# locuslab/qpth

Measured on AMD Instinct MI355X. Metric: QPs/sec (fwd+bwd) at batch=512 nz=100 nineq=100; 1/2/4/8 MI355X, higher is better.
Workload: dtype f64; 1 GPU; C2 fwd+bwd: batch=512 nz=100 nineq=100 neq=0 per GPU, dense random QP (prof-linear.py generator), QPFunction(verbose=-1) defaults, p requires grad; global_batch=512, parallelism=batch-sharded x1, tensor_dtype=f64, arithmetic=f64

## Files before the change

include/qpx.h:

```cpp
#ifndef QPX_H
#define QPX_H

#include <stddef.h>
#include <stdint.h>

#ifdef __cplusplus
extern "C" {
#endif

#define QPX_ABI_VERSION 8

enum { QPX_F32 = 0, QPX_F64 = 1, QPX_F32_WIDE = 2 };

enum {
    QPX_OK = 0,
    QPX_ERR_ARG = -1,
    QPX_ERR_UNSUPPORTED = -2,
    QPX_ERR_LAUNCH = -3,
    QPX_ERR_NO_DEVICE = -4
};

enum {
    QPX_ST_Q_NOT_SPD = 1,
    QPX_ST_A_RANK = 2,
// ... 15 lines not shown
int qpx_max_dim(void);
int qpx_supported(int dtype, int n, int m, int q);
enum { QPX_FAMILY_GRID = 1, QPX_FAMILY_TILE = 2, QPX_FAMILY_BIG = 3 };
int qpx_kernel_family(int dtype, int n, int m, int q);
int qpx_refine_supported(int dtype, int n, int m, int q);

int qpx_set_ipm_variant(int variant);
int qpx_get_ipm_variant(void);

int qpx_can_share_factors(int dtype, int n, int m, int q);

int qpx_big_gemm_r(int dtype, int B, int n, int m, int q, void* factors, qpx_stream_t stream);

int qpx_pre_factor(int dtype, int B, int n, int m, int q,
                   const void* Q, int64_t sQ, const void* G, int64_t sG, const void* A, int64_t sA,
                   void* factors, int32_t* status, qpx_stream_t stream);

int qpx_ipm(int dtype, int B, int n, int m, int q,
            const void* p, int64_t sp, const void* h, int64_t sh, const void* b, int64_t sb,
            void* factors, int64_t sfac, double eps, int maxIter, int notImprovedLim, int stall_policy,
            void* zhat, void* nu, void* lam, void* slack,
            int32_t* iters, int32_t* status, void* best_resid, void* trace, qpx_stream_t stream);

int qpx_forward(int dtype, int B, int n, int m, int q,
                const void* Q, int64_t sQ, const void* p, int64_t sp,
                const void* G, int64_t sG, const void* h, int64_t sh,
                const void* A, int64_t sA, const void* b, int64_t sb,
                void* factors, double eps, int maxIter, int notImprovedLim, int stall_policy,
                void* zhat, void* nu, void* lam, void* slack,
                int32_t* iters, int32_t* status, void* best_resid, void* trace, qpx_stream_t stream);

int qpx_factor_solve_kkt(int dtype, int B, int n, int m, int q, void* factors, int64_t sfac,
                         const void* d, const void* rx, const void* rs, const void* rz, const void* ry,
                         void* dx, void* ds, void* dz, void* dy,
                         int refine, const void* Q, int64_t sQ, const void* G, int64_t sG, const void* A, int64_t sA,
                         int32_t* status, qpx_stream_t stream);

int qpx_backward(int dtype, int B, int n, int m, int q, void* factors, int64_t sfac,
                 const void* zhat, const void* lam, const void* slack, const void* nu, const void* dl_dz,
                 void* dQ, void* dp, void* dG, void* dh, void* dA, void* db,
                 void* dx, void* dz, void* dy,
                 int refine, const void* Q, int64_t sQ, const void* G, int64_t sG, const void* A, int64_t sA,
                 int32_t* status, qpx_stream_t stream);

int qpx_backward_duals(int dtype, int B, int n, int m, int q, void* factors, int64_t sfac,
                       const void* zhat, const void* lam, const void* slack, const void* nu,
// ... 39 lines not shown
```

qpth_amd/_lib.py:

```python
import ctypes
import os

import torch

_HERE = os.path.dirname(os.path.abspath(__file__))
HIP_SO = os.path.join(_HERE, "libqpx_hip.so")

QPX_F32, QPX_F64, QPX_F32_WIDE = 0, 1, 2
ST_Q_NOT_SPD, ST_A_RANK, ST_KKT_BREAKDOWN, ST_INACCURATE, ST_MAXITER, ST_NONFINITE = 1, 2, 4, 8, 16, 32
STALL_OFF, STALL_REFERENCE, STALL_FLOOR = 0, 1, 2
FAMILY_GRID, FAMILY_TILE, FAMILY_BIG = 1, 2, 3

_vp, _i, _i64, _d = ctypes.c_void_p, ctypes.c_int, ctypes.c_int64, ctypes.c_double

_SIGNATURES = {
    "qpx_abi_version": (_i, []),
    "qpx_strerror": (ctypes.c_char_p, [_i]),
    "qpx_factor_elems": (ctypes.c_size_t, [_i, _i, _i, _i]),
    "qpx_max_dim": (_i, []),
    "qpx_supported": (_i, [_i, _i, _i, _i]),
    "qpx_kernel_family": (_i, [_i, _i, _i, _i]),
    "qpx_refine_supported": (_i, [_i, _i, _i, _i]),
    "qpx_set_ipm_variant": (_i, [_i]),
    "qpx_get_ipm_variant": (_i, []),
    "qpx_can_share_factors": (_i, [_i, _i, _i, _i]),
    "qpx_big_gemm_r": (_i, [_i, _i, _i, _i, _i, _vp, _vp]),
    "qpx_pre_factor": (_i, [_i, _i, _i, _i, _i, _vp, _i64, _vp, _i64, _vp, _i64, _vp, _vp, _vp]),
    "qpx_ipm": (_i, [_i, _i, _i, _i, _i, _vp, _i64, _vp, _i64, _vp, _i64, _vp, _i64, _d, _i, _i, _i,
                     _vp, _vp, _vp, _vp, _vp, _vp, _vp, _vp, _vp]),
    "qpx_forward": (_i, [_i, _i, _i, _i, _i, _vp, _i64, _vp, _i64, _vp, _i64, _vp, _i64, _vp, _i64,
                         _vp, _i64, _vp, _d, _i, _i, _i, _vp, _vp, _vp, _vp, _vp, _vp, _vp, _vp, _vp]),
    "qpx_factor_solve_kkt": (_i, [_i, _i, _i, _i, _i, _vp, _i64, _vp, _vp, _vp, _vp, _vp, _vp, _vp, _vp, _vp,
                                  _i, _vp, _i64, _vp, _i64, _vp, _i64, _vp, _vp]),
    "qpx_backward": (_i, [_i, _i, _i, _i, _i, _vp, _i64, _vp, _vp, _vp, _vp, _vp, _vp, _vp, _vp, _vp, _vp,
                          _vp, _vp, _vp, _vp, _i, _vp, _i64, _vp, _i64, _vp, _i64, _vp, _vp]),
    "qpx_backward_duals": (_i, [_i, _i, _i, _i, _i, _vp, _i64, _vp, _vp, _vp, _vp, _vp, _vp, _vp, _vp, _vp, _vp, _vp, _vp,
                                _vp, _vp, _vp, _vp, _i, _vp, _i64, _vp, _i64, _vp, _i64, _vp, _vp]),
    "qpx_jvp": (_i, [_i, _i, _i, _i, _i, _vp, _i64, _vp, _vp, _vp, _vp, _vp, _i64, _vp, _i64, _vp, _i64, _vp, _i64,
                     _vp, _i64, _vp, _i64, _vp, _vp, _vp, _vp, _i, _vp, _i64, _vp, _i64, _vp, _i64, _vp, _vp]),
    "qpx_multi_supported": (_i, [_i, _i, _i, _i]),
    "qpx_factor_solve_kkt_multi": (_i, [_i, _i, _i, _i, _i, _i, _vp, _i64, _vp, _vp, _vp, _vp, _vp, _vp, _vp, _vp, _vp, _vp, _vp]),
    "qpx_polish_supported": (_i, [_i, _i, _i, _i]),
    "qpx_polish": (_i, [_i, _i, _i, _i, _i, _vp, _i64, _vp, _i64, _vp, _i64, _vp, _i64, _vp, _i64, _vp, _i64,
                        _vp, _i64, _i, _i, _vp, _vp, _vp, _vp, _vp, _vp, _vp]),
    "qpx_batch_outer": (_i, [_i, _i, _i, _i, _vp, _vp, _vp, _vp, _d, _vp, _vp, ctypes.c_size_t, _vp]),
    "qpx_batch_outer_workspace_elems": (ctypes.c_size_t, [_i, _i, _i, _i]),
    "qpx_dense_solve": (_i, [_i, _i, _i, _vp, _vp, _vp, _vp]),
}
ABI_SYMBOLS = tuple(_SIGNATURES)


def _dtype_code(t):
# ... 45 lines not shown
    def __init__(self, path, strict=True):
        if not os.path.exists(path):
            raise RuntimeError(
                "qpth_amd: %s is missing. Build the gfx950 extension first "
                "(python -c 'import __graft_entry__ as g; g.build()' or qpth_amd/csrc/build.sh). "
                "There is no CPU fallback." % path)
        self.path = path
        self.dll = ctypes.CDLL(path)
        for name, (res, args) in _SIGNATURES.items():
            if not strict and not hasattr(self.dll, name):
                continue
            fn = getattr(self.dll, name)
            fn.restype, fn.argtypes = res, args
        if strict and self.dll.qpx_abi_version() != 8:
            raise RuntimeError("qpth_amd: ABI version mismatch in %s" % path)

    def check(self, code):
        if code != 0:
            raise RuntimeError("qpth_amd: %s (code %d)" % (self.dll.qpx_strerror(code).decode(), code))

    def factor_elems(self, dtype_code, n, m, q):
        return int(self.dll.qpx_factor_elems(dtype_code, n, m, q))

    def pre_factor(self, B, n, m, q, Q, G, A, factors, status, wide=False):
        Qp, Gp, Ap = Param(Q, 3), Param(G, 3), Param(A, 3)
        self.check(self.dll.qpx_pre_factor(
            _code(factors, wide), B, n, m, q, Qp.ptr, Qp.stride, Gp.ptr, Gp.stride, Ap.ptr, Ap.stride,
            _ptr(factors), _ptr(status), _stream(factors)))

    def ipm(self, B, n, m, q, p, h, b, factors, sfac, eps, maxIter, notImprovedLim, stall_policy,
            zhat, nu, lam, slack, iters, status, best_resid, trace=None, wide=False):
        pp, hp, bp = Param(p, 2), Param(h, 2), Param(b, 2)
        self.check(self.dll.qpx_ipm(
            _code(factors, wide), B, n, m, q, pp.ptr, pp.stride, hp.ptr, hp.stride, bp.ptr, bp.stride,
            _ptr(factors), int(sfac), float(eps), int(maxIter), int(notImprovedLim), int(stall_policy),
            _ptr(zhat), _ptr(nu), _ptr(lam), _ptr(slack), _ptr(iters), _ptr(status), _ptr(best_resid),
            _ptr(trace), _stream(factors)))

    def forward(self, B, n, m, q, Q, p, G, h, A, b, factors, eps, maxIter, notImprovedLim,
                stall_policy, zhat, nu, lam, slack, iters, status, best_resid, trace=None, wide=False):
        Qp, Gp, Ap = Param(Q, 3), Param(G, 3), Param(A, 3)
        pp, hp, bp = Param(p, 2), Param(h, 2), Param(b, 2)
        self.check(self.dll.qpx_forward(
            _code(factors, wide), B, n, m, q, Qp.ptr, Qp.stride, pp.ptr, pp.stride, Gp.ptr, Gp.stride,
            hp.ptr, hp.stride, Ap.ptr, Ap.stride, bp.ptr, bp.stride, _ptr(factors), float(eps),
            int(maxIter), int(notImprovedLim), int(stall_policy), _ptr(zhat), _ptr(nu), _ptr(lam),
            _ptr(slack), _ptr(iters), _ptr(status), _ptr(best_resid), _ptr(trace), _stream(factors)))

    def factor_solve_kkt(self, B, n, m, q, factors, sfac, d, rx, rs, rz, ry, dx, ds, dz, dy, status,
                         refine=0, Q=None, G=None, A=None, wide=False):
        Qp, Gp, Ap = Param(Q, 3), Param(G, 3), Param(A, 3)
        self.check(self.dll.qpx_factor_solve_kkt(
            _code(factors, wide), B, n, m, q, _ptr(factors), int(sfac), _ptr(d), _ptr(rx), _ptr(rs), _ptr(rz),
            _ptr(ry), _ptr(dx), _ptr(ds), _ptr(dz), _ptr(dy), int(refine), Qp.ptr, Qp.stride, Gp.ptr, Gp.stride,
            Ap.ptr, Ap.stride, _ptr(status), _stream(factors)))
# ... 82 lines not shown
```

qpth_amd/csrc/qpx_api.inc:

```
#include "qpx_forms.h"

namespace qpx {

constexpr int kMaxDim = 1024;
constexpr int kMaxDimPolish = 512;

static thread_local int g_grid_size = 0;
static thread_local int g_ipm_variant = 0;

inline bool use_grid(int n, int m, int q)
{
    return g_ipm_variant == 0 && grid_nb(n + q + m) > 0;
}

static thread_local int g_prefac_sweep = 0;
static thread_local int g_tile_nw = 0;
inline bool tile_chain(int nbt, int nw) { return (nbt == 7 || nbt == 4) && nw == 4; }
inline int tile_waves(int nbt, int B)
{
    int nw = g_tile_nw;
    if (nw == 0) nw = nbt == 7 ? 4 : (nbt == 4 && B <= 2 * 256 ? 4 : 1);
    if (nbt == 7 && nw == 1) nw = 2;
    if (nbt <= 2) nw = 1;
    if (nbt == 4 && nw > 2) nw = 4;
// ... 22 lines not shown
    if (d <= 256) return 4;
    if (d <= 512) return 8;
    if (d <= kMaxDim) return 16;
    return 0;
}

inline int check_dims(int dtype, int B, int n, int m, int q)
{
    if (dtype != QPX_F32 && dtype != QPX_F64 && dtype != QPX_F32_WIDE) return QPX_ERR_ARG;
    if (B < 1 || n < 1 || m < 1 || q < 0) return QPX_ERR_ARG;
    if (q > n) return QPX_ERR_ARG;
    if (!slots_for(n, m, q)) return QPX_ERR_UNSUPPORTED;
    return QPX_OK;
}

template <class T> inline size_t blob_elems(int n, int m, int q)
{
    const int images = blob_images<T>(n, m, q);
    return images == 8 ? big_layout(n, m, q).total : fac_layout(n, m, q, images).total;
}

#include "qpx_big_host.inc"

template <class T>
int api_pre_factor(int B, int n, int m, int q, const void* Q, int64_t sQ, const void* G, int64_t sG,
                   const void* A, int64_t sA, void* factors, int32_t* status, void* stream, int io32 = 0)
{
    if (!Q || !G || !factors || !status || (q > 0 && !A)) return QPX_ERR_ARG;
    PrefactorArgs<T> a;
    a.io32 = io32;
    a.B = B; a.n = n; a.m = m; a.q = q;
    a.Q = (const T*)Q; a.G = (const T*)G; a.A = (const T*)A;
    a.sQ = sQ; a.sG = sG; a.sA = sA;
    a.images = blob_images<T>(n, m, q);
    if (a.images == 8) {
        const size_t fs = big_layout(n, m, q).total;
        return big_split(B, stream, true, [&](int q0, int cnt, void* st, int part, int nparts) {
            return big_pre_factor<T>(cnt, n, m, q, advio(a.Q, (size_t)q0 * sQ, io32), sQ, advio(a.G, (size_t)q0 * sG, io32), sG,
                                     advio(a.A, (size_t)q0 * sA, io32), sA, (T*)factors + (size_t)q0 * fs, status + q0, st, io32);
        });
    }
    a.fac = (T*)factors; a.fac_stride = fac_layout(n, m, q, a.images).total; a.status = status;
    if constexpr (std::is_same<T, double>::value) {
        if (use_grid(n, m, q) && !g_prefac_sweep && prefac_tile_serves(n, m, q, a.images)) {
            const int nbn = tile_nb(n + q);
            const size_t pb = lds_elems_prefac_tile(nbn, (m + 15) / 16) * sizeof(double);
            prefac_deal(nbn, n + q, m, a.pf_k, a.pf_r);
#define QPX_PICK(NBN, EQ) if (nbn == NBN && (q > 0) == EQ) return launch_prefac_tile<NBN, EQ>(a, pb, stream);
            QPX_FORMS_PREFAC_TILE(QPX_PICK)
#undef QPX_PICK
        }
    }
    if (use_grid(n, m, q)) {
        const int nba = sweep_nb(n + q + m);
        const size_t gb = lds_elems_sweep(nba) * sizeof(T);
#define QPX_PICK(NBL) if (nba == NBL) return launch_sweep<T, NBL>(a, gb, stream);
        QPX_FORMS_SWEEP(QPX_PICK)
#undef QPX_PICK
    }
    return QPX_ERR_UNSUPPORTED;
}

template <class T>
int api_ipm(int B, int n, int m, int q, const void* p, int64_t sp, const void* h, int64_t sh,
            const void* bb, int64_t sb, void* factors, int64_t sfac, double eps, int maxIter, int notImprovedLim,
            int stall_policy, void* zhat, void* nu, void* lam, void* slack, int32_t* iters,
            int32_t* status, void* best_resid, void* trace, void* stream, int io32 = 0)
{
    if (!p || !h || !factors || !zhat || !lam || !slack || !iters || !status || !best_resid ||
        (q > 0 && (!nu || !bb)))
        return QPX_ERR_ARG;
    if (maxIter < 0 || stall_policy < 0 || stall_policy > 2) return QPX_ERR_ARG;
    IpmArgs<T> a;
    a.io32 = io32;
    a.B = B; a.n = n; a.m = m; a.q = q;
    a.p = (const T*)p; a.h = (const T*)h; a.b = (const T*)bb;
    a.sp = sp; a.sh = sh; a.sb = sb;
    a.fac = (T*)factors; a.fac_stride = (size_t)sfac;
    a.eps = (T)eps; a.maxIter = maxIter; a.notImprovedLim = notImprovedLim; a.stall_policy = stall_policy;
    a.zhat = (T*)zhat; a.nu = (T*)nu; a.lam = (T*)lam; a.slack = (T*)slack;
    a.iters = iters; a.status = status; a.best_resid = (T*)best_resid; a.trace = (T*)trace;
    a.images = blob_images<T>(n, m, q);
    if (a.images == 8) {
        if (sfac == 0 && B > 1) return QPX_ERR_ARG;
        return big_split(B, stream, a.trace == nullptr, [&](int q0, int cnt, void* st, int part, int nparts) {
            IpmArgs<T> s = a;
            const size_t o = (size_t)q0;
            s.B = cnt;
            s.p = advio(a.p, o * a.sp, io32); s.h = advio(a.h, o * a.sh, io32); s.b = advio(a.b, o * a.sb, io32);
            s.fac += o * a.fac_stride;
            s.zhat = advio(a.zhat, o * n, io32); s.lam = advio(a.lam, o * m, io32); s.slack = advio(a.slack, o * m, io32);
            s.nu = advio(a.nu, o * q, io32);
            s.iters += q0; s.status += q0; s.best_resid = advio(a.best_resid, o, io32);
            return big_ipm<T>(s, st, part, nparts);
        });
    }
    if (use_grid(n, m, q)) {
// ... 287 lines not shown
    if (!factors) return QPX_ERR_ARG;
    if (!qpx::use_big(n, m, q, dtype != QPX_F32 ? 8 : 4)) return QPX_ERR_UNSUPPORTED;
    return dtype != QPX_F32 ? qpx::big_gemm_r<double>(B, n, m, (double*)factors, stream, q)
                            : qpx::big_gemm_r<float>(B, n, m, (float*)factors, stream, q);
}

int qpx_can_share_factors(int dtype, int n, int m, int q)
{
    if (qpx::check_dims(dtype, 1, n, m, q) != QPX_OK) return 0;
    return qpx::use_big(n, m, q, dtype != QPX_F32 ? 8 : 4) ? 0 : 1;
}

int qpx_pre_factor(int dtype, int B, int n, int m, int q, const void* Q, int64_t sQ, const void* G,
                   int64_t sG, const void* A, int64_t sA, void* factors, int32_t* status,
                   qpx_stream_t stream)
{
    const int e = qpx::check_dims(dtype, B, n, m, q);
    if (e) return e;
    return dtype != QPX_F32
               ? qpx::api_pre_factor<double>(B, n, m, q, Q, sQ, G, sG, A, sA, factors, status, stream, dtype == QPX_F32_WIDE)
               : qpx::api_pre_factor<float>(B, n, m, q, Q, sQ, G, sG, A, sA, factors, status, stream);
}

int qpx_ipm(int dtype, int B, int n, int m, int q, const void* p, int64_t sp, const void* h,
            int64_t sh, const void* b, int64_t sb, void* factors, int64_t sfac, double eps, int maxIter,
            int notImprovedLim, int stall_policy, void* zhat, void* nu, void* lam, void* slack,
            int32_t* iters, int32_t* status, void* best_resid, void* trace, qpx_stream_t stream)
{
    const int e = qpx::check_dims(dtype, B, n, m, q);
    if (e) return e;
    return dtype != QPX_F32
               ? qpx::api_ipm<double>(B, n, m, q, p, sp, h, sh, b, sb, factors, sfac, eps, maxIter, notImprovedLim, stall_policy, zhat, nu, lam, slack, iters, status, best_resid, trace, stream, dtype == QPX_F32_WIDE)
               : qpx::api_ipm<float>(B, n, m, q, p, sp, h, sh, b, sb, factors, sfac, eps, maxIter, notImprovedLim, stall_policy, zhat, nu, lam, slack, iters, status, best_resid, trace, stream);
}

int qpx_forward(int dtype, int B, int n, int m, int q, const void* Q, int64_t sQ, const void* p,
                int64_t sp, const void* G, int64_t sG, const void* h, int64_t sh, const void* A,
                int64_t sA, const void* b, int64_t sb, void* factors, double eps, int maxIter,
                int notImprovedLim, int stall_policy, void* zhat, void* nu, void* lam, void* slack,
                int32_t* iters, int32_t* status, void* best_resid, void* trace, qpx_stream_t stream)
{
    int e = qpx_pre_factor(dtype, B, n, m, q, Q, sQ, G, sG, A, sA, factors, status, stream);
    if (e) return e;
    return qpx_ipm(dtype, B, n, m, q, p, sp, h, sh, b, sb, factors, (int64_t)qpx_factor_elems(dtype, n, m, q), eps, maxIter, notImprovedLim,
                   stall_policy, zhat, nu, lam, slack, iters, status, best_resid, trace, stream);
}
// ... 141 lines not shown
```

qpth_amd/csrc/qpx_grid.h:

```cpp
#pragma once
#include "qpx_forms.h"
#include "qpx_kernels.h"

namespace qpx {

template <int I0, int N, class F> QPX_DEV void static_for_(F&& f)
{
    if constexpr (I0 < N) {
        f(std::integral_constant<int, I0>{});
        static_for_<I0 + 1, N>(f);
    }
}
template <int N, class F> QPX_DEV void static_for(F&& f) { static_for_<0, N>(f); }

constexpr int gtri(int x) { return x * (x + 1) / 2; }
constexpr int gidx(int li, int lj) { return li * (li + 1) / 2 + lj; }

template <int GS> struct GridPos {
    int tid, a, b;
    static constexpr int NT = GS * GS;
    QPX_DEV explicit GridPos(const Block& blk) : tid(blk.tid), a(blk.tid % GS), b(blk.tid / GS) {}
    QPX_DEV void assign(const Block&, int*) {}
    QPX_DEV bool lead(const Block& blk) const { return blk.wave() == 0; }
    static QPX_DEV void sync(const Block& blk)
// ... 782 lines not shown

    const int lane = b.lane();
    const bool w0 = g.lead(b);
    const T mT = (T)m;
    const int io32 = a.io32;
    const In<T> pg(a.p, (size_t)qp * a.sp, io32), hg(a.h, (size_t)qp * a.sh, io32);
    const In<T> bg(q > 0 ? a.b : nullptr, (size_t)qp * a.sb, io32);

    if (a.status[qp] & (QPX_ST_Q_NOT_SPD | QPX_ST_A_RANK)) {
        const T nanv = Lim<T>::inf() - Lim<T>::inf();
        for (int i = b.tid; i < n; i += b.nt) put_(a.zhat, io32, (size_t)qp * n + i, nanv);
        for (int i = b.tid; i < m; i += b.nt) {
            put_(a.lam, io32, (size_t)qp * m + i, nanv);
            put_(a.slack, io32, (size_t)qp * m + i, nanv);
        }
        for (int i = b.tid; i < q; i += b.nt) put_(a.nu, io32, (size_t)qp * q + i, nanv);
        if (b.tid == 0) {
            a.iters[qp] = 0;
            put_(a.best_resid, io32, (size_t)qp, Lim<T>::inf());
        }
        return;
    }
    QPX_PROF_INIT
    for (int i = b.tid; i < n; i += NT) vP[i] = pg[i];
    for (int i = b.tid; i < M8; i += NT) {
        vC[i] = (i < m) ? hg[i] : T(0);
        vD[i] = T(1);
        vA[i] = T(1);
    }
    Mat::sync(b);
    block_matTvec2<T, 1, 0>(b, vC, F + lay.MT, m, vX0, F + lay.Kneg, n, vP, n);
    if (q > 0) {
        Mat::sync(b);
        for (int i = b.tid; i < q; i += NT) vTm[i] = bg[i];
        Mat::sync(b);
        for (int j = b.tid; j < m; j += NT) {
            T acc = vC[j];
            for (int r = 0; r < q; ++r) acc = fma_(-F[lay.W + (size_t)j * q + r], vTm[r], acc);
            vC[j] = acc;
        }
    }
    Mat::sync(b);
    QPX_PROF(0)

    typename Mat::Regs E;
    enum { kTau = 0, kBtau, kSigz, kSigs, kBres, kFeasPrev, kAlphaPrev, kMu, kSzdot, kFeas, kResid, kGt1 };
    enum { kStop = 0, kNnot, kFloor, kSt, kIters };
    if (b.tid == 0) {
        sc[kTau] = T(1); sc[kBtau] = T(1); sc[kSigz] = T(0); sc[kSigs] = T(0); sc[kBres] = Lim<T>::inf();
        sc[kFeasPrev] = T(0); sc[kAlphaPrev] = T(0);
        sc[kGt1] = F[lay.scal];
        ctrl[kStop] = 0; ctrl[kNnot] = 0; ctrl[kFloor] = 0; ctrl[kSt] = 0; ctrl[kIters] = 0;
    }
    for (int i = b.tid; i < M8; i += NT) {
        vZ[i] = T(1); vS[i] = T(1); vRZ[i] = T(1); vRS[i] = T(1);
// ... 1190 lines not shown
```

qpth_amd/csrc/qpx_kernels.h:

```cpp
#pragma once
#include "qpx_layout.h"
#include "qpx_platform.h"

#ifdef QPX_PROFILE
#define QPX_PROF_INIT long long qpx_prof_t = clock64(); long long qpx_prof_acc[8] = {0, 0, 0, 0, 0, 0, 0, 0};
#define QPX_PROF(i) { const long long qpx_prof_n = clock64(); qpx_prof_acc[i] += qpx_prof_n - qpx_prof_t; qpx_prof_t = qpx_prof_n; }
#define QPX_PROF_DUMP(ptr, T) if (b.tid == 0 && (ptr)) { for (int qpx_i = 0; qpx_i < 8; ++qpx_i) (ptr)[qpx_i] = (T)qpx_prof_acc[qpx_i]; }
#else
#define QPX_PROF_INIT
#define QPX_PROF(i)
#define QPX_PROF_DUMP(ptr, T)
#endif

namespace qpx {

template <class T> struct Lim;
template <> struct Lim<float> {
    static QPX_DEV float inf() { return __builtin_huge_valf(); }
    static QPX_DEV float tiny() { return 1.17549435e-38f; }
};
template <> struct Lim<double> {
    static QPX_DEV double inf() { return __builtin_huge_val(); }
    static QPX_DEV double tiny() { return 2.2250738585072014e-308; }
};
// ... 42 lines not shown
    {
        if (base) p = f32 ? reinterpret_cast<const T*>(reinterpret_cast<const float*>(base) + off) : base + off;
    }
    QPX_DEV explicit operator bool() const { return p != nullptr; }
    QPX_DEV T operator[](size_t i) const { return f32 ? (T) reinterpret_cast<const float*>(p)[i] : p[i]; }
};
template <class T> QPX_DEV void put_(T* base, int io32, size_t i, T v)
{
    if (sizeof(T) == 8 && io32) reinterpret_cast<float*>(base)[i] = (float)v;
    else base[i] = v;
}


template <class T> struct PrefactorArgs {
    int B, n, m, q;
    const T *Q, *G, *A;
    long long sQ, sG, sA;
    T* fac;
    size_t fac_stride;
    int* status;
    int images;
    int io32 = 0;
    unsigned pf_k[4] = {0, 0, 0, 0}, pf_r[4] = {0, 0, 0, 0};
};

template <class T> struct IpmArgs {
    int B, n, m, q;
    const T *p, *h, *b;
    long long sp, sh, sb;
    T* fac;
    size_t fac_stride;
    T eps;
    int maxIter, notImprovedLim, stall_policy;
    T *zhat, *nu, *lam, *slack;
    int *iters, *status;
    T* best_resid;
    T* trace;
    int images;
    int io32 = 0;
};

template <class T> struct KktArgs {
    int B, n, m, q;
    T* fac;
    size_t fac_stride;
    const T *d, *rx, *rs, *rz, *ry;
    T *dx, *ds, *dz, *dy;
    const T *zhat, *lam, *slack, *nu, *dl_dz;
    T *dQ, *dp, *dG, *dh, *dA, *db;
    int* status;
    int images;
    int refine;
    const T *Q, *G, *A;
    long long sQ, sG, sA;
    int io32 = 0;
    int jvp = 0;
    const T *tQ = nullptr, *tp = nullptr, *tG = nullptr, *th = nullptr, *tA = nullptr, *tb = nullptr;
    long long stQ = 0, stp = 0, stG = 0, sth = 0, stA = 0, stb = 0;
    const T *dl_dlam = nullptr, *dl_dnu = nullptr;
    int K = 0;
};

// ... 34 lines not shown
```

qpth_amd/csrc/qpx_layout.h:

```cpp
#pragma once
#include <cstddef>

namespace qpx {

#if defined(__HIPCC__)
#define QPX_LAYOUT_HD __host__ __device__ inline
#else
#define QPX_LAYOUT_HD inline
#endif

QPX_LAYOUT_HD size_t tri(size_t i) { return i * (i + 1) / 2; }
QPX_LAYOUT_HD int tri(int i) { return i * (i + 1) / 2; }
QPX_LAYOUT_HD size_t align4(size_t x) { return (x + 3) & ~(size_t)3; }

QPX_LAYOUT_HD int wave_nb(int m)
{
    const int need = (m + 7) / 8;
    if (need <= 2) return 2;
    if (need <= 4) return 4;
    if (need <= 8) return 8;
    if (need <= 13) return 13;
    return 0;
}

// ... 66 lines not shown
        f.scal = o;   o += 4;
        f.prof = o;   o += 8;
        f.T = o;      o += align4(tri((size_t)m));
    } else {
        f.nba = grid_nb(n + q + m);
        f.nbg = grid_nb(m);
        f.nbw = wave_nb(m);
        f.nbt = tile_nb(m);
        f.Kneg = o; o += align4((size_t)n * n);
        f.MT = o;   o += align4((size_t)n * m);
        f.NTn = o;  o += align4((size_t)q * n);
        f.W = o;    o += align4((size_t)m * q);
        f.S11i = o; o += align4((size_t)q * q);
        f.scal = o; o += 4;
        f.prof = o; o += 8;
        f.Rg = o;   if (images & 1) o += (size_t)(f.nbg * (f.nbg + 1) / 2) * 256;
        f.Rw = o;   if ((images & 2) && f.nbw > 0) o += (size_t)(f.nbw * (f.nbw + 1) / 2) * 64;
        f.Rm = o;   if ((images & 4) && f.nbt > 0) o += tile_image_elems(f.nbt);
    }
    f.total = o;
    return f;
}

enum : int {
    QPX_ST_Q_NOT_SPD = 1,
    QPX_ST_A_RANK = 2,
    QPX_ST_KKT_BREAKDOWN = 4,
    QPX_ST_INACCURATE = 8,
    QPX_ST_MAXITER = 16,
    QPX_ST_NONFINITE = 32
};

}
```

qpth_amd/csrc/qpx_prefac.h:

```cpp
#pragma once
#include <type_traits>

#include "qpx_tile.h"

namespace qpx {

constexpr int kPfVS = 16 * 17;
QPX_LAYOUT_HD constexpr int prefac_cap(int nbn) { return nbn == 7 ? 5 : 7; }
QPX_LAYOUT_HD constexpr size_t prefac_fixed_elems(int nbn) { return (size_t)16 * nbn + 8 + 7 * 16 * (size_t)nbn; }
QPX_LAYOUT_HD constexpr size_t lds_elems_prefac_tile(int nbn, int nbm = 1 << 20)
{
    const int slots = nbm < prefac_cap(nbn) ? nbm : prefac_cap(nbn);
    const size_t scr = tile_scratch_elems(nbn, 3, true), vs = (size_t)(nbn * (nbn + 1) / 2) * kPfVS,
                 yb = (size_t)slots * nbn * 256;
    const size_t u = scr > vs ? (scr > yb ? scr : yb) : (vs > yb ? vs : yb);
    return prefac_fixed_elems(nbn) + u;
}
QPX_LAYOUT_HD bool prefac_tile_serves(int n, int m, int q, int images)
{
    return images == 4 && n + q <= 112 && (tile_nb(n + q) == 4 || tile_nb(n + q) == 7) && tile_nb(m) > 0;
}

inline void prefac_deal(int nbn, int n, int m, unsigned (&pf_k)[4], unsigned (&pf_r)[4])
{
// ... 403 lines not shown
        }
#pragma unroll
        for (int r = 0; r < 4; ++r) acc[r] += acc2[r];
        r_store(i1, i2, acc);
    };
    const int nst = nbm < CAP ? nbm : CAP;
    if (nbm > CAP && iA >= CAP) {
#pragma unroll 1
        for (int i2 = 0; i2 < nst; ++i2) r_tile_reg(YA, iA, i2, i2);
        r_tile_reg(YA, iA, iA, -1);
    }
#pragma unroll 1
    for (unsigned rm = my_mask(a.pf_r); rm != 0; rm &= rm - 1) {
        const int t = __builtin_ctz(rm), i1 = tri_row(t);
        r_tile_lds(i1, t - i1 * (i1 + 1) / 2);
    }
    if (nbm - CAP == 2) {
        b.sync();
        if (w == 1) stage(YA, 0);
        b.sync();
        if (w == 0) r_tile_reg(YA, nbm - 1, nbm - 2, 0);
    }
    QPX_PROF(7)
    QPX_PROF_DUMP(F + lay.prof, T)
    if (b.tid == 0) a.status[qp] = 0;
}

}
```

qpth_amd/kkt.py:

```python
import contextlib
import threading

import numpy as np
import torch

from . import _lib

MULTI_RHS_BLOCK = 4

_STALL_POLICY = None


def set_stall_policy(policy):
    global _STALL_POLICY
    assert policy in (None, _lib.STALL_OFF, _lib.STALL_REFERENCE, _lib.STALL_FLOOR)
    _STALL_POLICY = policy


def default_stall_policy(B):
    if _STALL_POLICY is not None:
        return _STALL_POLICY
    return _lib.STALL_REFERENCE if B == 1 else _lib.STALL_FLOOR


# ... 41 lines not shown
                        still.append((ev, k, buf))
                self._pending = still
            lst = self._free.get(key)
            if lst:
                return key, lst.pop()
        if not may_allocate:
            return key, None
        return key, torch.zeros(count, dtype=torch.int32).pin_memory()

    def give(self, key, buf, event=None, keep=32):
        with self._lock:
            done = True if event is None else self._done(event)
            if not done:
                if done is not None and len(self._pending) < keep:
                    self._pending.append((event, key, buf))
                return
            lst = self._free.setdefault(key, [])
            if len(lst) < keep:
                lst.append(buf)


_PINNED = _PinnedPool()


class KKTFactors:
    @classmethod
    def build(cls, Q, G, A, nBatch=None, wide=False):
        self = cls()
        self.wide = bool(wide)
        if self.wide and Q.dtype != torch.float32:
            raise TypeError("qpth_amd: wide=True is for float32 tensors")
        B = nBatch if nBatch is not None else _batch_of(Q, G, A)
        self.B = B
        self.n = Q.size(-1)
        self.m = G.size(-2)
        self.q = A.size(-2) if (A is not None and A.nelement() > 0) else 0
        if G.size(-1) != self.n or Q.size(-2) != self.n or (self.q and A.size(-1) != self.n):
            raise RuntimeError("qpth_amd: inconsistent QP sizes Q%s G%s A%s" % (
                tuple(Q.shape), tuple(G.shape), tuple(A.shape) if A is not None else ()))
        for X, what in ((Q, "Q"), (G, "G"), (A if self.q else None, "A")):
            if X is None:
                continue
            if X.dtype != Q.dtype or X.device != Q.device:
                raise RuntimeError("qpth_amd: %s is %s on %s but Q is %s on %s (all of Q, p, G, h, A, b must share one "
                                   "dtype and one device)" % (what, X.dtype, X.device, Q.dtype, Q.device))
            if X.dim() not in (2, 3) or (X.dim() == 3 and X.size(0) not in (1, B)):
                raise RuntimeError("qpth_amd: %s has shape %s for a batch of %d" % (what, tuple(X.shape), B))
        self.lib = _lib.backend_for(Q)
        self.dtype, self.device = Q.dtype, Q.device
        self.Q, self.G, self.A = Q, G, (A if self.q else None)
        code = _lib.QPX_F32_WIDE if self.wide else (_lib.QPX_F64 if Q.dtype == torch.float64 else _lib.QPX_F32)
        self.elems = self.lib.factor_elems(code, self.n, self.m, self.q)
        self.variant = int(self.lib.dll.qpx_get_ipm_variant())
        self.refine_ok = bool(self.lib.dll.qpx_refine_supported(code, self.n, self.m, self.q)) if hasattr(self.lib.dll, "qpx_refine_supported") else True
        pcode = _lib.QPX_F64 if Q.dtype == torch.float64 else _lib.QPX_F32
        self.polish_ok = (not self.wide and hasattr(self.lib.dll, "qpx_polish_supported")
                          and bool(self.lib.dll.qpx_polish_supported(pcode, self.n, self.m, self.q)))
        share_ok = bool(self.lib.dll.qpx_can_share_factors(code, self.n, self.m, self.q))
        self.shared = B > 1 and share_ok and _is_shared(Q, B) and _is_shared(G, B) and _is_shared(A, B)
        nblob = 1 if self.shared else B
        self.sfac = 0 if self.shared else self.elems
        self.blob = torch.empty(nblob * self.elems, dtype=torch.float64 if self.wide else Q.dtype, device=Q.device)
        self.status = torch.empty(B, dtype=torch.int32, device=Q.device)
        with self._knob():
            self.lib.pre_factor(nblob, self.n, self.m, self.q, Q, G, A if self.q else None, self.blob, self.status,
                                wide=self.wide)
        if self.shared:
            self.status[1:] = self.status[0]
        self._pre_host = self._pre_event = self._pre_key = self._pre_bits = None
        if self.status.is_cuda:
            if not torch.cuda.is_current_stream_capturing():
                self._pre_key, self._pre_host = _PINNED.take(self.device, nblob)
            if self._pre_host is not None:
                self._pre_host.copy_(self.status[:nblob], non_blocking=True)
                self._pre_event = torch.cuda.Event()
                self._pre_event.record(torch.cuda.current_stream(self.device))
        return self

    def _release_pinned(self, done):
        host, key = self._pre_host, self._pre_key
        self._pre_host = self._pre_key = None
        if host is not None:
            _PINNED.give(key, host, None if done else self._pre_event)

    def __del__(self):
        try:
            if getattr(self, "_pre_host", None) is not None:
                self._release_pinned(False)
        except Exception:
            pass

    @contextlib.contextmanager
    def _knob(self):
        dll = self.lib.dll
        old = dll.qpx_set_ipm_variant(self.variant)
        guard = torch.cuda.device(self.device) if self.device.type == "cuda" else contextlib.nullcontext()
        try:
            with guard:
                yield
        finally:
# ... 37 lines not shown
            X = X.reshape(1, k).expand(self.B, k)
        return X.contiguous()

    def ipm(self, p, h, b, eps=1e-12, maxIter=20, notImprovedLim=3, stall_policy=None, want_trace=False):
        B, n, m, q = self.B, self.n, self.m, self.q
        dt, dev = self.dtype, self.device
        r = IpmResult()
        r.zhat = torch.empty(B, n, dtype=dt, device=dev)
        r.nu = torch.empty(B, q, dtype=dt, device=dev)
        r.lam = torch.empty(B, m, dtype=dt, device=dev)
        r.slacks = torch.empty(B, m, dtype=dt, device=dev)
        r.iters = torch.empty(B, dtype=torch.int32, device=dev)
        r.best_resid = torch.empty(B, dtype=dt, device=dev)
        r.trace = torch.full((maxIter, B, 3), float('nan'), dtype=dt, device=dev) if want_trace else None
        r.status = self.status
        if stall_policy is None:
            stall_policy = default_stall_policy(B)
        self._check(p, n, "p")
        self._check(h, m, "h")
        if q:
            if b is None or b.nelement() == 0:
                raise RuntimeError("qpth_amd: A has %d rows but b is empty" % q)
            self._check(b, q, "b")
        with self._knob():
            self.lib.ipm(B, n, m, q, p, h, b if q else None, self.blob, self.sfac, eps, maxIter, notImprovedLim,
                         stall_policy, r.zhat, r.nu if q else None, r.lam, r.slacks, r.iters, self.status,
                         r.best_resid, r.trace, wide=self.wide)
        return r

    def solve_kkt(self, d, rx, rs, rz, ry, refine=0):
        B, n, m, q = self.B, self.n, self.m, self.q
        dt, dev = self.dtype, self.device
        d = self._vec(d, m, "d")
        dx = torch.empty(B, n, dtype=dt, device=dev)
        ds = torch.empty(B, m, dtype=dt, device=dev)
        dz = torch.empty(B, m, dtype=dt, device=dev)
        dy = torch.empty(B, q, dtype=dt, device=dev) if q else None
        with self._knob():
            self.lib.factor_solve_kkt(B, n, m, q, self.blob, self.sfac, d, self._vec(rx, n, "rx"), self._vec(rs, m, "rs"),
                                      self._vec(rz, m, "rz"), self._vec(ry, q, "ry"), dx, ds, dz, dy, self.status,
                                      refine=refine, Q=self.Q, G=self.G, A=self.A, wide=self.wide)
        return dx, ds, dz, dy

    def _vecs(self, X, K, k, what):
        if X is None or X.nelement() == 0 or k == 0:
            return None
        if X.dtype != self.dtype or X.device != self.device:
            raise RuntimeError("qpth_amd: %s is %s on %s, the factors were built for %s on %s"
                               % (what, X.dtype, X.device, self.dtype, self.device))
        if tuple(X.shape) != (self.B, K, k):
# ... 132 lines not shown
```

qpth_amd/qp.py:

```python
from enum import Enum

import torch
from torch.autograd import Function

from . import _lib
from .kkt import KKTFactors
from .solvers.pdipm import batch as pdipm_b
from .util import expandParam, extract_nBatch


class QPSolvers(Enum):
    PDIPM_BATCHED = 1
    CVXPY = 2


def _print_trace(res):
    tr = res.trace.cpu()
    iters = res.iters.cpu()
    for i in range(int(iters.max().item())):
        row = tr[i][iters > i]
        print('iter: {}, pri_resid: {:.5e}, dual_resid: {:.5e}, mu: {:.5e}'.format(
            i, row[:, 0].mean(), row[:, 1].mean(), row[:, 2].mean()))


# ... 5 lines not shown

def QPFunction(eps=1e-12, verbose=0, notImprovedLim=3,
               maxIter=20, solver=QPSolvers.PDIPM_BATCHED,
               check_Q_spd=True, refine=None, duals=False):
    class QPFunctionFn(Function):
        @staticmethod
        def forward(ctx, Q_, p_, G_, h_, A_, b_):
            nBatch = extract_nBatch(Q_, p_, G_, h_, A_, b_)
            nineq, nz = G_.size(-2), G_.size(-1)
            neq = A_.size(-2) if A_.nelement() > 0 else 0
            ctx.wide = (solver == QPSolvers.PDIPM_BATCHED and refine is None and Q_.dtype == torch.float32
                        and f64_arithmetic_serves(nz, nineq, neq, _lib.backend_for(Q_)))
            Q, _ = expandParam(Q_, nBatch, 3)
            p, _ = expandParam(p_, nBatch, 2)
            G, _ = expandParam(G_, nBatch, 3)
            h, _ = expandParam(h_, nBatch, 2)
            A, _ = expandParam(A_, nBatch, 3)
            b, _ = expandParam(b_, nBatch, 2)

            assert(neq > 0 or nineq > 0)
            ctx.neq, ctx.nineq, ctx.nz = neq, nineq, nz

            if solver == QPSolvers.PDIPM_BATCHED:
                fac = KKTFactors.build(Q, G, A, nBatch, wide=ctx.wide)
                res = fac.ipm(p, h, b, eps, maxIter, notImprovedLim,
                              want_trace=(verbose == 1))
                ctx.refine = (2 if Q.dtype == torch.float32 and not ctx.wide else 0) if refine is None else int(refine)
                if ctx.refine > 0:
                    res = fac.polish(p, h, b, res, steps=ctx.refine, refine=0)
                fac.raise_on_failure(check_Q_spd)
                if verbose == 1:
                    _print_trace(res)
                if verbose >= 0:
                    if not bool((res.best_resid <= 1.).all().item()):
                        print(pdipm_b.INACC_ERR)
                ctx.fac = fac
                zhats, ctx.nus, ctx.lams, ctx.slacks = res.zhat, res.nu, res.lam, res.slacks
            elif solver == QPSolvers.CVXPY:
                from .solvers import external
                zhats, ctx.nus, ctx.lams, ctx.slacks = external.forward_batch(Q, p, G, h, A, b, neq)
                ctx.fac = None
                ctx.refine = 0 if refine is None else int(refine)
            else:
                assert False

            ctx.save_for_backward(zhats, Q_, p_, G_, h_, A_, b_)
            ctx.zhat = zhats.detach()
# ... 54 lines not shown
```

Baseline: 857,400 QPs/s.

## Precompute IPM initial-point constants in prefactor kernel and copy status on side stream

For f64 inequality-only grid problems, the prefactor kernel now also computes the IPM's initial matrix-vector products from p and h (the transformed h and the initial x) and stores them in a per-QP constants buffer. The IPM kernel reads these instead of recomputing its startup matTvec. Separately, the device-to-host copy of the prefactor status now runs on a side stream so it does not serialize with the main stream. The cost is an extra global buffer, more work in the prefactor tail, and identity checks to ensure the same p/h tensors are passed to ipm.

```diff
diff --git a/include/qpx.h b/include/qpx.h
--- a/include/qpx.h
+++ b/include/qpx.h
@@ -61,6 +61,18 @@
             void* zhat, void* nu, void* lam, void* slack,
             int32_t* iters, int32_t* status, void* best_resid, void* trace, qpx_stream_t stream);
 
+int qpx_prefac_forms_consts(int dtype, int n, int m, int q);
+size_t qpx_consts_elems(int n, int m);
+int qpx_pre_factor_consts(int dtype, int B, int n, int m, int q,
+                          const void* Q, int64_t sQ, const void* G, int64_t sG, const void* A, int64_t sA,
+                          const void* p, int64_t sp, const void* h, int64_t sh, const void* b, int64_t sb,
+                          void* factors, void* consts, int32_t* status, qpx_stream_t stream);
+int qpx_ipm_consts(int dtype, int B, int n, int m, int q,
+                   const void* p, int64_t sp, const void* h, int64_t sh, const void* b, int64_t sb,
+                   void* factors, int64_t sfac, const void* consts, double eps, int maxIter, int notImprovedLim,
+                   int stall_policy, void* zhat, void* nu, void* lam, void* slack,
+                   int32_t* iters, int32_t* status, void* best_resid, void* trace, qpx_stream_t stream);
+
 int qpx_forward(int dtype, int B, int n, int m, int q,
                 const void* Q, int64_t sQ, const void* p, int64_t sp,
                 const void* G, int64_t sG, const void* h, int64_t sh,
diff --git a/qpth_amd/_lib.py b/qpth_amd/_lib.py
--- a/qpth_amd/_lib.py
+++ b/qpth_amd/_lib.py
@@ -28,6 +28,12 @@
     "qpx_pre_factor": (_i, [_i, _i, _i, _i, _i, _vp, _i64, _vp, _i64, _vp, _i64, _vp, _vp, _vp]),
     "qpx_ipm": (_i, [_i, _i, _i, _i, _i, _vp, _i64, _vp, _i64, _vp, _i64, _vp, _i64, _d, _i, _i, _i,
                      _vp, _vp, _vp, _vp, _vp, _vp, _vp, _vp, _vp]),
+    "qpx_prefac_forms_consts": (_i, [_i, _i, _i, _i]),
+    "qpx_consts_elems": (ctypes.c_size_t, [_i, _i]),
+    "qpx_pre_factor_consts": (_i, [_i, _i, _i, _i, _i, _vp, _i64, _vp, _i64, _vp, _i64, _vp, _i64, _vp, _i64, _vp, _i64,
+                                   _vp, _vp, _vp, _vp]),
+    "qpx_ipm_consts": (_i, [_i, _i, _i, _i, _i, _vp, _i64, _vp, _i64, _vp, _i64, _vp, _i64, _vp, _d, _i, _i, _i,
+                            _vp, _vp, _vp, _vp, _vp, _vp, _vp, _vp, _vp]),
     "qpx_forward": (_i, [_i, _i, _i, _i, _i, _vp, _i64, _vp, _i64, _vp, _i64, _vp, _i64, _vp, _i64,
                          _vp, _i64, _vp, _d, _i, _i, _i, _vp, _vp, _vp, _vp, _vp, _vp, _vp, _vp, _vp]),
     "qpx_factor_solve_kkt": (_i, [_i, _i, _i, _i, _i, _vp, _i64, _vp, _vp, _vp, _vp, _vp, _vp, _vp, _vp, _vp,
@@ -119,15 +125,29 @@
     def factor_elems(self, dtype_code, n, m, q):
         return int(self.dll.qpx_factor_elems(dtype_code, n, m, q))
 
-    def pre_factor(self, B, n, m, q, Q, G, A, factors, status, wide=False):
-        Qp, Gp, Ap = Param(Q, 3), Param(G, 3), Param(A, 3)
+    def pre_factor(self, B, n, m, q, Q, G, A, factors, status, wide=False, p=None, h=None, b=None, consts=None):
+        Qp, Gp, Ap = Param(Q, 3), Param(G, 3), Param(A, 3)
+        if consts is not None:
+            pp, hp, bp = Param(p, 2), Param(h, 2), Param(b, 2)
+            self.check(self.dll.qpx_pre_factor_consts(
+                _code(factors, wide), B, n, m, q, Qp.ptr, Qp.stride, Gp.ptr, Gp.stride, Ap.ptr, Ap.stride,
+                pp.ptr, pp.stride, hp.ptr, hp.stride, bp.ptr, bp.stride, _ptr(factors), _ptr(consts), _ptr(status),
+                _stream(factors)))
+            return
         self.check(self.dll.qpx_pre_factor(
             _code(factors, wide), B, n, m, q, Qp.ptr, Qp.stride, Gp.ptr, Gp.stride, Ap.ptr, Ap.stride,
             _ptr(factors), _ptr(status), _stream(factors)))
 
     def ipm(self, B, n, m, q, p, h, b, factors, sfac, eps, maxIter, notImprovedLim, stall_policy,
-            zhat, nu, lam, slack, iters, status, best_resid, trace=None, wide=False):
+            zhat, nu, lam, slack, iters, status, best_resid, trace=None, wide=False, consts=None):
         pp, hp, bp = Param(p, 2), Param(h, 2), Param(b, 2)
+        if consts is not None:
+            self.check(self.dll.qpx_ipm_consts(
+                _code(factors, wide), B, n, m, q, pp.ptr, pp.stride, hp.ptr, hp.stride, bp.ptr, bp.stride,
+                _ptr(factors), int(sfac), _ptr(consts), float(eps), int(maxIter), int(notImprovedLim), int(stall_policy),
+                _ptr(zhat), _ptr(nu), _ptr(lam), _ptr(slack), _ptr(iters), _ptr(status), _ptr(best_resid),
+                _ptr(trace), _stream(factors)))
+            return
         self.check(self.dll.qpx_ipm(
             _code(factors, wide), B, n, m, q, pp.ptr, pp.stride, hp.ptr, hp.stride, bp.ptr, bp.stride,
             _ptr(factors), int(sfac), float(eps), int(maxIter), int(notImprovedLim), int(stall_policy),
diff --git a/qpth_amd/csrc/qpx_api.inc b/qpth_amd/csrc/qpx_api.inc
--- a/qpth_amd/csrc/qpx_api.inc
+++ b/qpth_amd/csrc/qpx_api.inc
@@ -68,13 +68,25 @@
 
 #include "qpx_big_host.inc"
 
+template <class T> inline bool prefac_forms_consts(int n, int m, int q)
+{
+    return std::is_same<T, double>::value && q == 0 && use_grid(n, m, q) && !g_prefac_sweep &&
+           prefac_tile_serves(n, m, q, blob_images<T>(n, m, q));
+}
+
 template <class T>
 int api_pre_factor(int B, int n, int m, int q, const void* Q, int64_t sQ, const void* G, int64_t sG,
-                   const void* A, int64_t sA, void* factors, int32_t* status, void* stream, int io32 = 0)
+                   const void* A, int64_t sA, void* factors, int32_t* status, void* stream, int io32 = 0,
+                   const void* p = nullptr, int64_t sp = 0, const void* h = nullptr, int64_t sh = 0, void* consts = nullptr)
 {
     if (!Q || !G || !factors || !status || (q > 0 && !A)) return QPX_ERR_ARG;
     PrefactorArgs<T> a;
     a.io32 = io32;
+    if (consts && prefac_forms_consts<T>(n, m, q)) {
+        if (!p || !h) return QPX_ERR_ARG;
+        a.p = (const T*)p; a.h = (const T*)h; a.sp = sp; a.sh = sh;
+        a.consts = (T*)consts; a.consts_stride = consts_elems(n, m);
+    }
     a.B = B; a.n = n; a.m = m; a.q = q;
     a.Q = (const T*)Q; a.G = (const T*)G; a.A = (const T*)A;
     a.sQ = sQ; a.sG = sG; a.sA = sA;
@@ -111,14 +123,16 @@
 int api_ipm(int B, int n, int m, int q, const void* p, int64_t sp, const void* h, int64_t sh,
             const void* bb, int64_t sb, void* factors, int64_t sfac, double eps, int maxIter, int notImprovedLim,
             int stall_policy, void* zhat, void* nu, void* lam, void* slack, int32_t* iters,
-            int32_t* status, void* best_resid, void* trace, void* stream, int io32 = 0)
+            int32_t* status, void* best_resid, void* trace, void* stream, int io32 = 0, const void* consts = nullptr)
 {
     if (!p || !h || !factors || !zhat || !lam || !slack || !iters || !status || !best_resid ||
         (q > 0 && (!nu || !bb)))
         return QPX_ERR_ARG;
     if (maxIter < 0 || stall_policy < 0 || stall_policy > 2) return QPX_ERR_ARG;
+    if (consts && !prefac_forms_consts<T>(n, m, q)) return QPX_ERR_UNSUPPORTED;
     IpmArgs<T> a;
     a.io32 = io32;
+    a.consts = (const T*)consts; a.consts_stride = consts ? consts_elems(n, m) : 0;
     a.B = B; a.n = n; a.m = m; a.q = q;
     a.p = (const T*)p; a.h = (const T*)h; a.b = (const T*)bb;
     a.sp = sp; a.sh = sh; a.sb = sb;
@@ -452,6 +466,37 @@
                : qpx::api_pre_factor<float>(B, n, m, q, Q, sQ, G, sG, A, sA, factors, status, stream);
 }
 
+int qpx_prefac_forms_consts(int dtype, int n, int m, int q)
+{
+    if (qpx::check_dims(dtype, 1, n, m, q) != QPX_OK) return 0;
+    return dtype != QPX_F32 && qpx::prefac_forms_consts<double>(n, m, q) ? 1 : 0;
+}
+
+size_t qpx_consts_elems(int n, int m) { return n < 1 || m < 1 ? 0 : qpx::consts_elems(n, m); }
+
+int qpx_pre_factor_consts(int dtype, int B, int n, int m, int q, const void* Q, int64_t sQ, const void* G, int64_t sG,
+                          const void* A, int64_t sA, const void* p, int64_t sp, const void* h, int64_t sh, const void* b,
+                          int64_t sb, void* factors, void* consts, int32_t* status, qpx_stream_t stream)
+{
+    (void)b; (void)sb;
+    const int e = qpx::check_dims(dtype, B, n, m, q);
+    if (e) return e;
+    if (!consts || !qpx_prefac_forms_consts(dtype, n, m, q)) return qpx_pre_factor(dtype, B, n, m, q, Q, sQ, G, sG, A, sA, factors, status, stream);
+    return qpx::api_pre_factor<double>(B, n, m, q, Q, sQ, G, sG, A, sA, factors, status, stream, dtype == QPX_F32_WIDE, p, sp, h, sh, consts);
+}
+
+int qpx_ipm_consts(int dtype, int B, int n, int m, int q, const void* p, int64_t sp, const void* h, int64_t sh, const void* b,
+                   int64_t sb, void* factors, int64_t sfac, const void* consts, double eps, int maxIter, int notImprovedLim,
+                   int stall_policy, void* zhat, void* nu, void* lam, void* slack, int32_t* iters, int32_t* status,
+                   void* best_resid, void* trace, qpx_stream_t stream)
+{
+    const int e = qpx::check_dims(dtype, B, n, m, q);
+    if (e) return e;
+    return dtype != QPX_F32
+               ? qpx::api_ipm<double>(B, n, m, q, p, sp, h, sh, b, sb, factors, sfac, eps, maxIter, notImprovedLim, stall_policy, zhat, nu, lam, slack, iters, status, best_resid, trace, stream, dtype == QPX_F32_WIDE, consts)
+               : qpx::api_ipm<float>(B, n, m, q, p, sp, h, sh, b, sb, factors, sfac, eps, maxIter, notImprovedLim, stall_policy, zhat, nu, lam, slack, iters, status, best_resid, trace, stream, 0, consts);
+}
+
 int qpx_ipm(int dtype, int B, int n, int m, int q, const void* p, int64_t sp, const void* h,
             int64_t sh, const void* b, int64_t sb, void* factors, int64_t sfac, double eps, int maxIter,
             int notImprovedLim, int stall_policy, void* zhat, void* nu, void* lam, void* slack,
diff --git a/qpth_amd/csrc/qpx_grid.h b/qpth_amd/csrc/qpx_grid.h
--- a/qpth_amd/csrc/qpx_grid.h
+++ b/qpth_amd/csrc/qpx_grid.h
@@ -828,15 +828,20 @@
         return;
     }
     QPX_PROF_INIT
-    for (int i = b.tid; i < n; i += NT) vP[i] = pg[i];
+    const T* cst = a.consts ? a.consts + (size_t)qp * a.consts_stride : nullptr;
+    const int mc = consts_c_elems(m);
+    if (!cst)
+        for (int i = b.tid; i < n; i += NT) vP[i] = pg[i];
     for (int i = b.tid; i < M8; i += NT) {
-        vC[i] = (i < m) ? hg[i] : T(0);
+        vC[i] = cst ? (i < mc ? cst[i] : T(0)) : ((i < m) ? hg[i] : T(0));
         vD[i] = T(1);
         vA[i] = T(1);
     }
+    if (cst)
+        for (int i = b.tid; i < n; i += NT) vX0[i] = cst[mc + i];
     Mat::sync(b);
-    block_matTvec2<T, 1, 0>(b, vC, F + lay.MT, m, vX0, F + lay.Kneg, n, vP, n);
-    if (q > 0) {
+    if (!cst) block_matTvec2<T, 1, 0>(b, vC, F + lay.MT, m, vX0, F + lay.Kneg, n, vP, n);
+    if (q > 0 && !cst) {
         Mat::sync(b);
         for (int i = b.tid; i < q; i += NT) vTm[i] = bg[i];
         Mat::sync(b);
diff --git a/qpth_amd/csrc/qpx_kernels.h b/qpth_amd/csrc/qpx_kernels.h
--- a/qpth_amd/csrc/qpx_kernels.h
+++ b/qpth_amd/csrc/qpx_kernels.h
@@ -88,6 +88,10 @@
     int images;
     int io32 = 0;
     unsigned pf_k[4] = {0, 0, 0, 0}, pf_r[4] = {0, 0, 0, 0};
+    const T *p = nullptr, *h = nullptr;
+    long long sp = 0, sh = 0;
+    T* consts = nullptr;
+    size_t consts_stride = 0;
 };
 
 template <class T> struct IpmArgs {
@@ -104,6 +108,8 @@
     T* trace;
     int images;
     int io32 = 0;
+    const T* consts = nullptr;
+    size_t consts_stride = 0;
 };
 
 template <class T> struct KktArgs {
diff --git a/qpth_amd/csrc/qpx_layout.h b/qpth_amd/csrc/qpx_layout.h
--- a/qpth_amd/csrc/qpx_layout.h
+++ b/qpth_amd/csrc/qpx_layout.h
@@ -112,6 +112,9 @@
     return f;
 }
 
+QPX_LAYOUT_HD int consts_c_elems(int m) { return 16 * ((m + 15) / 16); }
+QPX_LAYOUT_HD size_t consts_elems(int n, int m) { return (size_t)consts_c_elems(m) + (size_t)n; }
+
 enum : int {
     QPX_ST_Q_NOT_SPD = 1,
     QPX_ST_A_RANK = 2,
diff --git a/qpth_amd/csrc/qpx_prefac.h b/qpth_amd/csrc/qpx_prefac.h
--- a/qpth_amd/csrc/qpx_prefac.h
+++ b/qpth_amd/csrc/qpx_prefac.h
@@ -449,6 +449,27 @@
         if (w == 0) r_tile_reg(YA, nbm - 1, nbm - 2, 0);
     }
     QPX_PROF(7)
+    if constexpr (!kEq) {
+        if (a.consts) {
+            T* pv = rd;
+            T* xv = gpart;
+            T* hv = gpart + MPN;
+            const In<T> pg(a.p, (size_t)qp * a.sp, a.io32), hg(a.h, (size_t)qp * a.sh, a.io32);
+            T ph;
+            if (b.tid < 128) ph = b.tid < n ? pg[b.tid] : T(0);
+            else ph = b.tid - 128 < m ? hg[b.tid - 128] : T(0);
+            b.sync();
+            if (b.tid < MPN) pv[b.tid] = ph;
+            if (b.tid >= 128 && b.tid < 128 + 112) hv[b.tid - 128] = ph;
+            b.sync();
+            block_matTvec2<T, 1, 0>(b, hv, F + lay.MT, m, xv, F + lay.Kneg, n, pv, n);
+            b.sync();
+            T* cst = a.consts + (size_t)qp * a.consts_stride;
+            const int mc = consts_c_elems(m);
+            for (int i = b.tid; i < mc; i += b.nt) cst[i] = i < m ? hv[i] : T(0);
+            for (int i = b.tid; i < n; i += b.nt) cst[mc + i] = xv[i];
+        }
+    }
     QPX_PROF_DUMP(F + lay.prof, T)
     if (b.tid == 0) a.status[qp] = 0;
 }
diff --git a/qpth_amd/kkt.py b/qpth_amd/kkt.py
--- a/qpth_amd/kkt.py
+++ b/qpth_amd/kkt.py
@@ -87,10 +87,21 @@
 
 _PINNED = _PinnedPool()
 
+_SIDE_LOCK = threading.Lock()
+_SIDE_STREAMS = {}
+
+
+def _side_stream(device):
+    with _SIDE_LOCK:
+        st = _SIDE_STREAMS.get(device.index)
+        if st is None:
+            st = _SIDE_STREAMS[device.index] = torch.cuda.Stream(device)
+        return st
+
 
 class KKTFactors:
     @classmethod
-    def build(cls, Q, G, A, nBatch=None, wide=False):
+    def build(cls, Q, G, A, nBatch=None, wide=False, p=None, h=None, b=None):
         self = cls()
         self.wide = bool(wide)
         if self.wide and Q.dtype != torch.float32:
@@ -127,20 +138,37 @@
         self.sfac = 0 if self.shared else self.elems
         self.blob = torch.empty(nblob * self.elems, dtype=torch.float64 if self.wide else Q.dtype, device=Q.device)
         self.status = torch.empty(B, dtype=torch.int32, device=Q.device)
-        with self._knob():
+        self.consts = self._consts_p = self._consts_h = self._consts_b = None
+        pre_done = None
+        with self._knob():
+            if (p is not None and h is not None and not self.shared and hasattr(self.lib.dll, "qpx_prefac_forms_consts")
+                    and self.lib.dll.qpx_prefac_forms_consts(code, self.n, self.m, self.q)
+                    and self._fits(p, self.n) and self._fits(h, self.m)):
+                ce = int(self.lib.dll.qpx_consts_elems(self.n, self.m))
+                self.consts = torch.empty(B * ce, dtype=self.blob.dtype, device=Q.device)
+                self._consts_p, self._consts_h, self._consts_b = p, h, b
             self.lib.pre_factor(nblob, self.n, self.m, self.q, Q, G, A if self.q else None, self.blob, self.status,
-                                wide=self.wide)
+                                wide=self.wide, p=p, h=h, b=b if self.q else None, consts=self.consts)
+            if self.status.is_cuda and not torch.cuda.is_current_stream_capturing():
+                pre_done = torch.cuda.Event()
+                pre_done.record(torch.cuda.current_stream(self.device))
         if self.shared:
             self.status[1:] = self.status[0]
         self._pre_host = self._pre_event = self._pre_key = self._pre_bits = None
-        if self.status.is_cuda:
-            if not torch.cuda.is_current_stream_capturing():
-                self._pre_key, self._pre_host = _PINNED.take(self.device, nblob)
-            if self._pre_host is not None:
+        if pre_done is not None:
+            self._pre_key, self._pre_host = _PINNED.take(self.device, nblob)
+            side = _side_stream(self.device)
+            side.wait_event(pre_done)
+            self.status.record_stream(side)
+            with torch.cuda.stream(side):
                 self._pre_host.copy_(self.status[:nblob], non_blocking=True)
-                self._pre_event = torch.cuda.Event()
-                self._pre_event.record(torch.cuda.current_stream(self.device))
+            self._pre_event = torch.cuda.Event()
+            self._pre_event.record(side)
         return self
+
+    def _fits(self, X, k):
+        return (X.dtype == self.dtype and X.device == self.device and
+                tuple(X.shape) in ((k,), (self.B, k), (1, k)))
 
     def _release_pinned(self, done):
         host, key = self._pre_host, self._pre_key
@@ -224,10 +252,12 @@
             if b is None or b.nelement() == 0:
                 raise RuntimeError("qpth_amd: A has %d rows but b is empty" % q)
             self._check(b, q, "b")
+        consts = self.consts if (self.consts is not None and p is self._consts_p and h is self._consts_h
+                                 and (not q or b is self._consts_b)) else None
         with self._knob():
             self.lib.ipm(B, n, m, q, p, h, b if q else None, self.blob, self.sfac, eps, maxIter, notImprovedLim,
                          stall_policy, r.zhat, r.nu if q else None, r.lam, r.slacks, r.iters, self.status,
-                         r.best_resid, r.trace, wide=self.wide)
+                         r.best_resid, r.trace, wide=self.wide, consts=consts)
         return r
 
     def solve_kkt(self, d, rx, rs, rz, ry, refine=0):
diff --git a/qpth_amd/qp.py b/qpth_amd/qp.py
--- a/qpth_amd/qp.py
+++ b/qpth_amd/qp.py
@@ -51,7 +51,7 @@
             ctx.neq, ctx.nineq, ctx.nz = neq, nineq, nz
 
             if solver == QPSolvers.PDIPM_BATCHED:
-                fac = KKTFactors.build(Q, G, A, nBatch, wide=ctx.wide)
+                fac = KKTFactors.build(Q, G, A, nBatch, wide=ctx.wide, p=p, h=h, b=b)
                 res = fac.ipm(p, h, b, eps, maxIter, notImprovedLim,
                               want_trace=(verbose == 1))
                 ctx.refine = (2 if Q.dtype == torch.float32 and not ctx.wide else 0) if refine is None else int(refine)
```

Result: slower. 848,100 QPs/s (-1.1%).
